# liyheng/MAGPO

Measured on AMD Instinct MI355X. Metric: env-steps/sec (all agents stepping jointly), CoordSum-4ag, full MAGPO update loop, higher is better.
Workload: dtype f32 (fp32 MFMA; as bf16 x3 operand splits = 24 mantissa bits, six products, fp32 accumulate: the GRU forward scan's recurrent GEMM)

## Files before the change

magpo_amd/csrc/seg_fused.hip:

```cpp
#include "fm_rows.hpp"

namespace magpo {

struct SegArgs {
  int tail;
  long R; int K;
  const float* r; const float* gp; long ldg; const float* gamma; const float* beta;
  const float* wo_t; const float* res; const float* s1; const float* s2;
  const float* pe; const int* pos; int npos;
  float* u; float* y; float* o; float* ope;
  const float* w0_t; const float* b0; float* out0; long ld0;
  const float* hs; const float* hw; const float* hb1; float* value;
  const float* q2_t[4]; float* q2[4]; int nq2;
  float* hn; const float* w1_t; const float* b1; float* logits;
  const int* rows;
};

__device__ __forceinline__ Row row_rms_reg(const Row& x, const Row& s) {
  Row q;
#pragma unroll
  for (int j = 0; j < 16; ++j) q.v[j] = x.v[j] * x.v[j];
  const float rstd = rsqrtf(row_sum(q) * (1.0f / 64.0f) + EPSN);
  Row r;
#pragma unroll
  for (int j = 0; j < 16; ++j) r.v[j] = x.v[j] * rstd * s.v[j];
  return r;
}

__device__ __forceinline__ Row dense64_reg(const Row& x, const float4 (&w)[4][4], const float* __restrict__ bias, int kq) {
  Row y;
#pragma unroll
  for (int g = 0; g < 4; ++g) {
    f32x4 acc = {0.f, 0.f, 0.f, 0.f};
#pragma unroll
    for (int gk = 0; gk < 4; ++gk) {
      acc = __builtin_amdgcn_mfma_f32_16x16x4f32(w[g][gk].x, x.v[4 * gk], acc, 0, 0, 0);
      acc = __builtin_amdgcn_mfma_f32_16x16x4f32(w[g][gk].y, x.v[4 * gk + 1], acc, 0, 0, 0);
      acc = __builtin_amdgcn_mfma_f32_16x16x4f32(w[g][gk].z, x.v[4 * gk + 2], acc, 0, 0, 0);
      acc = __builtin_amdgcn_mfma_f32_16x16x4f32(w[g][gk].w, x.v[4 * gk + 3], acc, 0, 0, 0);
    }
    float4 b = make_float4(0.f, 0.f, 0.f, 0.f);
    if (bias) b = ld4g(bias + 16 * g + 4 * kq);
    y.v[4 * g] = acc[0] + b.x; y.v[4 * g + 1] = acc[1] + b.y; y.v[4 * g + 2] = acc[2] + b.z; y.v[4 * g + 3] = acc[3] + b.w;
  }
  return y;
}
constexpr int WSP = 68;
__device__ __forceinline__ Row dense64_lds(const Row& x, const float* __restrict__ ws, int m, int kq) {
  Row y;
#pragma unroll
  for (int g = 0; g < 4; ++g) {
    f32x4 acc = {0.f, 0.f, 0.f, 0.f};
#pragma unroll
    for (int gk = 0; gk < 4; ++gk) {
      const float4 w = *reinterpret_cast<const float4*>(ws + (16 * g + m) * WSP + 16 * gk + 4 * kq);
      acc = __builtin_amdgcn_mfma_f32_16x16x4f32(w.x, x.v[4 * gk], acc, 0, 0, 0);
      acc = __builtin_amdgcn_mfma_f32_16x16x4f32(w.y, x.v[4 * gk + 1], acc, 0, 0, 0);
      acc = __builtin_amdgcn_mfma_f32_16x16x4f32(w.z, x.v[4 * gk + 2], acc, 0, 0, 0);
      acc = __builtin_amdgcn_mfma_f32_16x16x4f32(w.w, x.v[4 * gk + 3], acc, 0, 0, 0);
    }
    y.v[4 * g] = acc[0]; y.v[4 * g + 1] = acc[1]; y.v[4 * g + 2] = acc[2]; y.v[4 * g + 3] = acc[3];
  }
  return y;
}
__device__ __forceinline__ void load_w64(float4 (&w)[4][4], const float* __restrict__ Wt, int m, int kq) {
#pragma unroll
  for (int g = 0; g < 4; ++g)
#pragma unroll
    for (int gk = 0; gk < 4; ++gk) w[g][gk] = ld4g(Wt + (long)(16 * g + m) * AE + 16 * gk + 4 * kq);
}

template <int TAIL>
__global__ __launch_bounds__(64, 1) void k_seg_post(SegArgs a) {
  const int lane = threadIdx.x, m = lane & 15, kq = lane >> 4;
  const long ntiles = (a.R + 15) >> 4;
  float4 wo[4][4], w0[4][4], w0b[TAIL != 0 ? 4 : 1][4], w0c[TAIL == 2 ? 4 : 1][4];
  load_w64(wo, a.wo_t, m, kq);
  if (TAIL == 1 || TAIL == 3) load_w64(w0, a.w0_t, m, kq);
  if constexpr (TAIL == 1) { if (a.nq2 > 0) load_w64(w0b, a.q2_t[0], m, kq); }
  Row b1r;
  if constexpr (TAIL == 3) {
    load_w64(w0b, a.w1_t, m, kq);
#pragma unroll
    for (int j = 0; j < 16; ++j) { const int n = 16 * (j >> 2) + 4 * kq + (j & 3); b1r.v[j] = n < a.K ? a.b1[n] : 0.f; }
  }
  if (TAIL == 2) {
    load_w64(w0, a.w0_t, m, kq);
#pragma unroll
    for (int g = 0; g < 4; ++g)
#pragma unroll
      for (int gk = 0; gk < 4; ++gk) {
        w0b[g][gk] = ld4g(a.w0_t + (long)(64 + 16 * g + m) * AE + 16 * gk + 4 * kq);
        w0c[g][gk] = ld4g(a.w0_t + (long)(128 + 16 * g + m) * AE + 16 * gk + 4 * kq);
      }
  }
  const Row gam = row_load(a.gamma, kq), bet = row_load(a.beta, kq);
// ... 5 lines not shown
  const float hb1 = TAIL == 1 ? a.hb1[0] : 0.f;
  auto rowc = [&](long tile) { return min(tile * 16 + m, a.R - 1); };
  long tile = blockIdx.x;
  Row nr, ng, nres, npe;
  const bool want_pe = a.ope || TAIL == 1 || TAIL == 2;
  auto pe_row = [&](long row) {
    int p = a.pos[row];
    p = p < 0 ? 0 : (p >= a.npos ? a.npos - 1 : p);
    return row_load(a.pe + (long)p * AE, kq);
  };
  auto src_row = [&](long row) { return a.rows ? (long)a.rows[row] : row; };
  {
    const long row = rowc(tile), src = src_row(row);
    nr = row_load(a.r + row * AE, kq); ng = row_load(a.gp + src * a.ldg, kq); nres = row_load(a.res + src * AE, kq);
    if (want_pe) npe = pe_row(row);
  }
  for (; tile < ntiles; tile += gridDim.x) {
    const long row = tile * 16 + m;
    const long rw = min(row, a.R - 1);
    const Row r = nr, g = ng, res = nres, per = npe;
    {
      const long nrow = rowc(min(tile + (long)gridDim.x, ntiles - 1)), nsrc = src_row(nrow);
      nr = row_load(a.r + nrow * AE, kq); ng = row_load(a.gp + nsrc * a.ldg, kq); nres = row_load(a.res + nsrc * AE, kq);
      if (want_pe) npe = pe_row(nrow);
    }
    Row sq;
#pragma unroll
    for (int j = 0; j < 16; ++j) sq.v[j] = r.v[j] * r.v[j];
    const float mu = row_sum(r) * (1.0f / 64.0f), m2 = row_sum(sq) * (1.0f / 64.0f);
    const float rstd = rsqrtf(fmaxf(m2 - mu * mu, 0.f) + EPSN);
    Row u;
#pragma unroll
    for (int j = 0; j < 16; ++j) u.v[j] = fswish(g.v[j]) * ((r.v[j] - mu) * rstd * gam.v[j] + bet.v[j]);
    row_store(a.u + rw * AE, kq, u);
    const Row y = dense64_reg(u, wo, nullptr, kq);
    if (a.y) row_store(a.y + rw * AE, kq, y);
    Row o = row_add(res, y);
    {
      Row q;
#pragma unroll
      for (int j = 0; j < 16; ++j) q.v[j] = o.v[j] * o.v[j];
      const float rs = rsqrtf(row_sum(q) * (1.0f / 64.0f) + EPSN);
#pragma unroll
      for (int j = 0; j < 16; ++j) o.v[j] = o.v[j] * rs * s1.v[j];
    }
    if (a.s2) o = row_rms_reg(o, s2r);
    if (a.o) row_store(a.o + rw * AE, kq, o);
    Row ope = o;
    if (want_pe) {
      ope = row_add(o, per);
      if (a.ope) row_store(a.ope + rw * AE, kq, ope);
    }
    if (TAIL == 1) {
      const Row hv = row_add(dense64_reg(o, w0, nullptr, kq), b0r);
      row_store(a.out0 + rw * a.ld0, kq, hv);
      const Row hn = row_rms_reg(row_gelu(hv), hsr);
      Row hw;
#pragma unroll
      for (int j = 0; j < 16; ++j) hw.v[j] = hn.v[j] * hwr.v[j];
      const float val = row_sum(hw) + hb1;
      a.value[rw] = val;
      if constexpr (TAIL == 1) {
        if (a.nq2 > 0) row_store(a.q2[0] + rw * AE, kq, dense64_reg(ope, w0b, nullptr, kq));
      }
      for (int k = 1; k < a.nq2; ++k) {
        const Row q2 = dense64(ope, a.q2_t[k], nullptr, m, kq);
        row_store(a.q2[k] + rw * AE, kq, q2);
// ... 1 lines not shown
    } else if (TAIL == 2) {
      float* orow = a.out0 + rw * a.ld0;
      if constexpr (TAIL == 2) {
        row_store(orow, kq, dense64_reg(ope, w0, nullptr, kq));
        row_store(orow + 64, kq, dense64_reg(ope, w0b, nullptr, kq));
        row_store(orow + 128, kq, dense64_reg(ope, w0c, nullptr, kq));
      }
    } else if (TAIL == 3) {
      const Row hp = row_add(dense64_reg(o, w0, nullptr, kq), b0r);
      row_store(a.out0 + rw * a.ld0, kq, hp);
      const Row hn = row_rms_reg(row_gelu(hp), hsr);
      row_store(a.hn + rw * AE, kq, hn);
      if constexpr (TAIL == 3) {
        Row lg = row_add(dense64_reg(hn, w0b, nullptr, kq), b1r);
#pragma unroll
        for (int j = 0; j < 16; ++j) { const int n = 16 * (j >> 2) + 4 * kq + (j & 3); lg.v[j] = n < a.K ? lg.v[j] : 0.f; }
        row_store(a.logits + rw * AE, kq, lg);
      }
    }
  }
}


struct SegBwdArgs {
  long R;
  const float* a; const float* y; const float* s1; const float* s2;
  const float* d0; const float* d1; const float* d2;
  const float* wo_nat;
  const float* wo_t;
  const float* r; const float* gp; long ldg; const float* gamma; const float* beta;
  float* dsum; float* dr; float* dgp; long lddg;
  float* slab_s1; float* slab_s2; float* slab_ga; float* slab_be;
  const int* rows;
};

template <bool RECOMP>
__global__ __launch_bounds__(64, 1) void k_seg_bwd(SegBwdArgs a) {
  const int lane = threadIdx.x, m = lane & 15, kq = lane >> 4;
  const long ntiles = (a.R + 15) >> 4;
  float4 wo[4][4];
  __shared__ __align__(16) float wot[RECOMP ? 64 * WSP : 4];
  load_w64(wo, a.wo_nat, m, kq);
  constexpr bool recompute = RECOMP;
  if (recompute) {
    for (int i = lane; i < 64 * 16; i += 64) *reinterpret_cast<float4*>(&wot[(i >> 4) * WSP + 4 * (i & 15)]) = ld4g(a.wo_t + (i >> 4) * AE + 4 * (i & 15));
    __syncthreads();
  }
  __shared__ __align__(16) float prm[RECOMP ? 4 * 64 : 4];
  Row s1_, s2_, gam_, bet_;
  if (!RECOMP) {
    s1_ = row_load(a.s1, kq); gam_ = row_load(a.gamma, kq); bet_ = row_load(a.beta, kq);
    if (a.s2) s2_ = row_load(a.s2, kq);
  } else {
    prm[lane] = a.s1[lane]; prm[64 + lane] = a.s2 ? a.s2[lane] : 0.f; prm[128 + lane] = a.gamma[lane]; prm[192 + lane] = a.beta[lane];
    __syncthreads();
  }
  auto prow = [&](int which, const Row& reg) -> Row {
    if (!RECOMP) return reg;
    int off = which * 64 + 4 * kq;
    asm volatile("" : "+v"(off));
    Row r;
#pragma unroll
    for (int g = 0; g < 4; ++g) {
      const float4 t4 = *reinterpret_cast<const float4*>(&prm[off + 16 * g]);
      r.v[4 * g] = t4.x; r.v[4 * g + 1] = t4.y; r.v[4 * g + 2] = t4.z; r.v[4 * g + 3] = t4.w;
    }
    return r;
  };
  Row ds1, ds2, dga, dbe;
#pragma unroll
  for (int j = 0; j < 16; ++j) { ds1.v[j] = 0.f; ds2.v[j] = 0.f; dga.v[j] = 0.f; dbe.v[j] = 0.f; }
  auto rowc = [&](long tile) { return min(tile * 16 + m, a.R - 1); };
  Row na, ny, nd, nd1, nd2, nr, ng;
  auto fetch = [&](long row) {
    const long src = a.rows ? (long)a.rows[row] : row;
    na = row_load(a.a + src * AE, kq);
    if (a.y && !recompute) ny = row_load(a.y + row * AE, kq);
    nd = row_load(a.d0 + row * AE, kq);
    if (a.d1) nd1 = row_load(a.d1 + row * AE, kq);
    if (a.d2) nd2 = row_load(a.d2 + row * AE, kq);
    nr = row_load(a.r + row * AE, kq);
    ng = row_load(a.gp + src * a.ldg, kq);
  };
  long tile = blockIdx.x;
  fetch(rowc(tile));
  for (; tile < ntiles; tile += gridDim.x) {
    const long row = tile * 16 + m;
    const long rw = min(row, a.R - 1);
    const float live = row < a.R ? 1.f : 0.f;
    Row x = (a.y && !recompute) ? row_add(na, ny) : na;
    Row d = nd;
    if (a.d1) d = row_add(d, nd1);
    if (a.d2) d = row_add(d, nd2);
    const Row r = nr, g = ng;
    fetch(rowc(min(tile + (long)gridDim.x, ntiles - 1)));
    Row t;
#pragma unroll
    for (int j = 0; j < 16; ++j) t.v[j] = r.v[j] * r.v[j];
    const float mu = row_sum(r) * (1.0f / 64.0f), m2 = row_sum(t) * (1.0f / 64.0f);
    const float rstd = rsqrtf(fmaxf(m2 - mu * mu, 0.f) + EPSN);
    if (recompute) {
      const Row gam = prow(2, gam_), bet = prow(3, bet_);
      Row u;
#pragma unroll
      for (int j = 0; j < 16; ++j) u.v[j] = fswish(g.v[j]) * ((r.v[j] - mu) * rstd * gam.v[j] + bet.v[j]);
      x = row_add(x, dense64_lds(u, wot, m, kq));
    }
#pragma unroll
    for (int j = 0; j < 16; ++j) t.v[j] = x.v[j] * x.v[j];
    const float rstd1 = rsqrtf(row_sum(t) * (1.0f / 64.0f) + EPSN);
    Row xh1;
#pragma unroll
    for (int j = 0; j < 16; ++j) xh1.v[j] = x.v[j] * rstd1;
    const Row s1 = prow(0, s1_);
    if (a.s2) {
      const Row s2 = prow(1, s2_);
      Row y1;
#pragma unroll
      for (int j = 0; j < 16; ++j) { y1.v[j] = xh1.v[j] * s1.v[j]; t.v[j] = y1.v[j] * y1.v[j]; }
      const float rstd2 = rsqrtf(row_sum(t) * (1.0f / 64.0f) + EPSN);
#pragma unroll
      for (int j = 0; j < 16; ++j) {
        const float xh2 = y1.v[j] * rstd2;
        ds2.v[j] += live * d.v[j] * xh2;
        y1.v[j] = xh2;
        d.v[j] = d.v[j] * s2.v[j];
        t.v[j] = d.v[j] * xh2;
      }
      const float dot2 = row_sum(t) * (1.0f / 64.0f);
#pragma unroll
      for (int j = 0; j < 16; ++j) d.v[j] = (d.v[j] - y1.v[j] * dot2) * rstd2;
    }
#pragma unroll
    for (int j = 0; j < 16; ++j) {
      ds1.v[j] += live * d.v[j] * xh1.v[j];
      d.v[j] = d.v[j] * s1.v[j];
      t.v[j] = d.v[j] * xh1.v[j];
    }
    const float dot1 = row_sum(t) * (1.0f / 64.0f);
    Row dsum;
#pragma unroll
    for (int j = 0; j < 16; ++j) dsum.v[j] = (d.v[j] - xh1.v[j] * dot1) * rstd1;
    row_store(a.dsum + rw * AE, kq, dsum);
    const Row du = dense64_reg(dsum, wo, nullptr, kq);
    const Row gam = prow(2, gam_), bet = prow(3, bet_);
    Row xh, gg, dg;
#pragma unroll
    for (int j = 0; j < 16; ++j) {
      xh.v[j] = (r.v[j] - mu) * rstd;
      const float rn = xh.v[j] * gam.v[j] + bet.v[j];
      const float sg = fast_sigmoid(g.v[j]);
      const float sw = g.v[j] * sg;
      const float swg = sg * (1.0f + g.v[j] * (1.0f - sg));
      const float drn = du.v[j] * sw;
      dg.v[j] = du.v[j] * rn * swg;
      dga.v[j] += live * drn * xh.v[j];
      dbe.v[j] += live * drn;
      gg.v[j] = drn * gam.v[j];
      t.v[j] = gg.v[j] * xh.v[j];
    }
    const float mg = row_sum(gg) * (1.0f / 64.0f), mgx = row_sum(t) * (1.0f / 64.0f);
    Row dx;
#pragma unroll
    for (int j = 0; j < 16; ++j) dx.v[j] = (gg.v[j] - mg - xh.v[j] * mgx) * rstd;
    row_store(a.dr + rw * AE, kq, dx);
    row_store(a.dgp + rw * a.lddg, kq, dg);
  }
#pragma unroll
  for (int j = 0; j < 16; ++j) { ds1.v[j] = gsum(ds1.v[j], 16); ds2.v[j] = gsum(ds2.v[j], 16); dga.v[j] = gsum(dga.v[j], 16); dbe.v[j] = gsum(dbe.v[j], 16); }
  if (m == 0) {
    row_store(a.slab_s1 + (long)blockIdx.x * AE, kq, ds1);
    if (a.s2) row_store(a.slab_s2 + (long)blockIdx.x * AE, kq, ds2);
    row_store(a.slab_ga + (long)blockIdx.x * AE, kq, dga);
    row_store(a.slab_be + (long)blockIdx.x * AE, kq, dbe);
  }
}

}

using namespace magpo;

extern "C" int magpo_seg_post(const int* dims_host, long R, const void* const* p, int nptrs, hipStream_t st) {
  if (R <= 0) return MAGPO_OK;
  if (nptrs != 34) { set_error("magpo_seg_post: pointer table size mismatch"); return MAGPO_EINVAL; }
  SegArgs a;
  a.tail = dims_host[0]; a.K = dims_host[1]; a.npos = dims_host[2]; a.ldg = dims_host[3]; a.ld0 = dims_host[4]; a.nq2 = dims_host[5];
  a.R = R;
  if (a.tail < 0 || a.tail > 3 || a.nq2 < 0 || a.nq2 > 4 || a.K < 1 || a.K > 64) { set_error("magpo_seg_post: bad arguments"); return MAGPO_EINVAL; }
  int i = 0;
  a.r = (const float*)p[i++]; a.gp = (const float*)p[i++]; a.gamma = (const float*)p[i++]; a.beta = (const float*)p[i++];
  a.wo_t = (const float*)p[i++]; a.res = (const float*)p[i++]; a.s1 = (const float*)p[i++]; a.s2 = (const float*)p[i++];
  a.pe = (const float*)p[i++]; a.pos = (const int*)p[i++];
  a.u = (float*)p[i++]; a.y = (float*)p[i++]; a.o = (float*)p[i++]; a.ope = (float*)p[i++];
  a.w0_t = (const float*)p[i++]; a.b0 = (const float*)p[i++]; a.out0 = (float*)p[i++];
  a.hs = (const float*)p[i++]; a.hw = (const float*)p[i++]; a.hb1 = (const float*)p[i++]; a.value = (float*)p[i++];
  for (int k = 0; k < 4; ++k) a.q2_t[k] = (const float*)p[i++];
  for (int k = 0; k < 4; ++k) a.q2[k] = (float*)p[i++];
  a.hn = (float*)p[i++]; a.w1_t = (const float*)p[i++]; a.b1 = (const float*)p[i++]; a.logits = (float*)p[i++];
  a.rows = (const int*)p[i++];
  const long ntiles = (R + 15) / 16;
  long grid = 256 * 4;
  if (grid > ntiles) grid = ntiles;
  switch (a.tail) {
    case 0: hipLaunchKernelGGL(k_seg_post<0>, dim3((unsigned)grid), dim3(64), 0, st, a); break;
    case 1: hipLaunchKernelGGL(k_seg_post<1>, dim3((unsigned)grid), dim3(64), 0, st, a); break;
    case 2: hipLaunchKernelGGL(k_seg_post<2>, dim3((unsigned)grid), dim3(64), 0, st, a); break;
    default: hipLaunchKernelGGL(k_seg_post<3>, dim3((unsigned)grid), dim3(64), 0, st, a); break;
  }
  return check_launch("magpo_seg_post");
}

extern "C" int magpo_seg_bwd_grid(long R) { const long nt = (R + 15) / 16; return (int)(nt < 1024 ? (nt < 1 ? 1 : nt) : 1024); }

extern "C" int magpo_seg_bwd(long R, long ldg, long lddg, const void* const* p, int nptrs, hipStream_t st) {
  if (R <= 0) return MAGPO_OK;
  if (nptrs != 21) { set_error("magpo_seg_bwd: pointer table size mismatch"); return MAGPO_EINVAL; }
  SegBwdArgs a;
  a.R = R; a.ldg = ldg; a.lddg = lddg;
  int i = 0;
  a.a = (const float*)p[i++]; a.y = (const float*)p[i++]; a.s1 = (const float*)p[i++]; a.s2 = (const float*)p[i++];
  a.d0 = (const float*)p[i++]; a.d1 = (const float*)p[i++]; a.d2 = (const float*)p[i++]; a.wo_nat = (const float*)p[i++];
  a.r = (const float*)p[i++]; a.gp = (const float*)p[i++]; a.gamma = (const float*)p[i++]; a.beta = (const float*)p[i++];
  a.dsum = (float*)p[i++]; a.dr = (float*)p[i++]; a.dgp = (float*)p[i++];
  a.slab_s1 = (float*)p[i++]; a.slab_s2 = (float*)p[i++]; a.slab_ga = (float*)p[i++]; a.slab_be = (float*)p[i++];
  a.rows = (const int*)p[i++];
  a.wo_t = (const float*)p[i++];
  if (a.wo_t) hipLaunchKernelGGL(k_seg_bwd<true>, dim3((unsigned)magpo_seg_bwd_grid(R)), dim3(64), 0, st, a);
  else hipLaunchKernelGGL(k_seg_bwd<false>, dim3((unsigned)magpo_seg_bwd_grid(R)), dim3(64), 0, st, a);
  return check_launch("magpo_seg_bwd");
}
```

magpo_amd/sable.py:

```python
from __future__ import annotations

import math
from typing import Dict, Optional, Tuple

import numpy as np
import torch

from ._lib import lib
from .params import FlatParams, WidthEmbedding, guider_layout, guider_named_views, init_guider
from .tuning import Tuning

E = 64
TILE = 64
LW = 64


def decay_kappas(n_head: int, scaling: float):
    k = 1.0 - np.exp(np.linspace(np.log(np.float32(1 / 32)), np.log(np.float32(1 / 512)), n_head, dtype=np.float32))
    return [float(x) for x in (k.astype(np.float32) * np.float32(scaling)).astype(np.float32)]


class _Bufs:
    def __init__(self, device):
        self.device = device
# ... 415 lines not shown
                        v[d + "retn2.gn.scale"], v[d + "retn2.gn.bias"],
                        g(f"qkvg1_{k}", 4 * E), g(f"q2_{k}"), g(f"kvg2_{k}", 4 * E)]
            tabs = (np.array([N, A, K, F, nb, nh, self.hs, self.gs, self.npos, 1 if value_only else 0, self.Fld, self.tuning.act_envs_per_wave,
                              1 if pending else 0, 1 if flush else 0, 1 if precand else 0, 1 if defer else 0], dtype=np.int32),
                    np.array((self.kappas + [0.0] * 4)[:4], dtype=np.float32),
                    np.array([ptr(t) for t in glob], dtype=np.uint64), np.array([ptr(t) for t in blk], dtype=np.uint64))
            if len(self._act_tabs) > 4096:
                self._act_tabs.clear()
            self._act_tabs[cache_key] = tabs
        dims, kap, gp, bp = tabs
        keys = None
        if kdev is None and not value_only:
            keys = np.ascontiguousarray(np.asarray(sample_keys, dtype=np.uint32).reshape(A, 2))
        self.L.call("magpo_sable_act", dims.ctypes.data, kap.ctypes.data, None if keys is None else keys.ctypes.data,
                    gp.ctypes.data, int(gp.size), bp.ctypes.data, int(bp.size), self._st())

    get_actions = act_fused

    def _seg_post(self, tail, r, gp, ldg, gamma, beta, wo_t, res, s1, s2, pos, u, y, o, ope, R, w0_t=None, b0=None, out0=None, ld0=0,
                  hs=None, hw=None, hb1=None, value=None, q2_t=(), q2=(), hn=None, w1_t=None, b1=None, logits=None, rows=None):
        ptr = lambda t: 0 if t is None else t.data_ptr()
        q2_t, q2 = list(q2_t) + [None] * (4 - len(q2_t)), list(q2) + [None] * (4 - len(q2))
        tab = [r, gp, gamma, beta, wo_t, res, s1, s2, self.pe, pos, u, y, o, ope, w0_t, b0, out0, hs, hw, hb1, value, *q2_t, *q2, hn, w1_t, b1, logits, rows]
        key = (tail, R, tuple(ptr(t) for t in tab))
        ent = self._seg_tabs.get(key)
        if ent is None:
            nq2 = sum(1 for t in q2 if t is not None)
            ent = (np.array([tail, self.K, self.npos, ldg, ld0, nq2], dtype=np.int32), np.array([ptr(t) for t in tab], dtype=np.uint64))
            if len(self._seg_tabs) > 256:
                self._seg_tabs.clear()
            self._seg_tabs[key] = ent
        self.L.call("magpo_seg_post", ent[0].ctypes.data, R, ent[1].ctypes.data, int(ent[1].size), self._st())

    def _seg_bwd(self, a, y, s1, s2, d0, d1, d2, wo_nat, r, gp, ldg, pfx, dsum, dr, dgp, lddg, R, g_s1, g_s2, acc_s1=False, rows=None, wo_t=None):
        v, gv, b = self.v, self.gv, self.b
        ptr = lambda t: 0 if t is None else t.data_ptr()
        G = self.L.call("magpo_seg_bwd_grid", R)
        sl = [b.get(f"sb_{i}", (G, E)) for i in range(4)]
        tab = [a, y, s1, s2, d0, d1, d2, wo_nat, r, gp, v[pfx + "gn.scale"], v[pfx + "gn.bias"], dsum, dr, dgp, sl[0], sl[1] if s2 is not None else None, sl[2], sl[3], rows, wo_t]
        key = ("bwd", R, ldg, lddg, tuple(ptr(t) for t in tab))
        ent = self._seg_tabs.get(key)
        if ent is None:
            ent = np.array([ptr(t) for t in tab], dtype=np.uint64)
            self._seg_tabs[key] = ent
        self.L.call("magpo_seg_bwd", R, ldg, lddg, ent.ctypes.data, int(ent.size), self._st())
        self.reduce(sl[0], g_s1, accumulate=acc_s1)
        if s2 is not None:
            self.reduce(sl[1], g_s2)
        self.reduce(sl[2], gv[pfx + "gn.scale"]); self.reduce(sl[3], gv[pfx + "gn.bias"])

    def train_fwd(self, obs, prev_idx, pos, dones, s0, seq_env, nseq: int, T: int, classes=None):
        L, st, A, K, F, v, b, nb, E = self.L, self._st(), self.A, self.K, self.F, self.v, self.b, self.nb, self.E
        R = nseq * T * A
        g = lambda n, w=E: b.get("t_" + n, (R, w))
        direct = classes is not None and self.fused_segments
        self._saved = dict(obs=obs, prev_idx=prev_idx, pos=pos, dones=dones, nseq=nseq, T=T, R=R, classes=classes, direct=direct)
        rep, reppe, hv, value = g("rep"), g("reppe"), g("hv"), b.get("t_value", (R,))
        logits = b.get("t_logits", (R, LW), zero=True)
        if classes is not None:
            obs_c, pos_c = classes["rows"][0], classes["rows"][1]
            Ce = obs_c.shape[0]
            xn_c, kin_c, qkvg_c = b.get("c_xn0", (Ce, E)), b.get("c_kin0", (Ce, E)), b.get("c_qkvg0", (Ce, 4 * E))
            L.call("magpo_embed_fwd", 0, obs_c, F, F, v["enc.obs.norm.scale"], v["enc.obs.dense.kernel"], None, 0, v["enc.ln.scale"],
                   self.pe, pos_c, 1, self.npos, None, 0, xn_c, E, kin_c, E, Ce, E, st)
            self.lin(kin_c, E, self.wt["qkvg0"], None, qkvg_c, 4 * E, Ce, E, 4 * E)
            if not direct:
                L.call("magpo_gather_rows", xn_c, E, classes["enc"][0], g("xn0"), E, R, E, st)
                L.call("magpo_gather_rows", qkvg_c, 4 * E, classes["enc"][0], g("qkvg0", 4 * E), 4 * E, R, 4 * E, st)
        elif self.wide:
            on, z0 = b.get("t_on", (R, 128)), g("z0")
            L.call("magpo_obsnorm_fwd", obs, self.Fld, F, v["enc.obs.norm.scale"], on, R, st)
            self.lin(on, 128, self.wt["wobs"], None, z0, E, R, 128, E)
            L.call("magpo_headmid_fwd", z0, E, v["enc.ln.scale"], g("xn0"), E, None, None, None, 0, R, E, st)
            L.call("magpo_add_pe", g("xn0"), E, self.pe, pos, 1, self.npos, g("kin0"), E, R, E, st)
        else:
            L.call("magpo_embed_fwd", 0, obs, self.Fld, F, v["enc.obs.norm.scale"], v["enc.obs.dense.kernel"], None, 0, v["enc.ln.scale"],
                   self.pe, pos, 1, self.npos, None, 0, g("xn0"), E, g("kin0"), E, R, E, st)
        for k in range(nb):
            e = f"enc.block{k}."
            rows = classes["enc"][0] if direct and k == 0 else None
            if rows is not None:
                xn, qkvg = xn_c, qkvg_c
            else:
                xn, qkvg = g(f"xn{k}"), g(f"qkvg{k}", 4 * E)
            r, u = g(f"r{k}"), g(f"u{k}")
            y = None if self.fused_segments else g(f"y{k}")
            if k > 0 or classes is None:
                self.lin(g(f"kin{k}"), E, self.wt[f"qkvg{k}"], None, qkvg, 4 * E, R, E, 4 * E)
            self._ret_fwd(qkvg, 4 * E, qkvg[:, E:], 4 * E, qkvg[:, 2 * E:], 4 * E, r, s0[0][k], seq_env, dones, f"st_e{k}", nseq, T, 0, rows=rows)
            if self.fused_segments and k == nb - 1:
                self._seg_post(1, r, qkvg[:, 3 * E:], 4 * E, v[e + "retn.gn.scale"], v[e + "retn.gn.bias"], self.wt[f"wo{k}"], xn,
                               v[e + "ln1.scale"], v[e + "ln2.scale"], pos, u, y, rep, reppe, R, w0_t=self.wt["vh0"], b0=v["enc.head.dense0.bias"],
                               out0=hv, ld0=E, hs=v["enc.head.norm.scale"], hw=v["enc.head.dense1.kernel"], hb1=v["enc.head.dense1.bias"],
                               value=value, q2_t=[self.wt[f"q2{j}"] for j in range(nb)], q2=[g(f"q2{j}") for j in range(nb)], rows=rows)
                continue
            if self.fused_segments:
                repb = g(f"repb{k}")
                self._seg_post(0, r, qkvg[:, 3 * E:], 4 * E, v[e + "retn.gn.scale"], v[e + "retn.gn.bias"], self.wt[f"wo{k}"], xn,
                               v[e + "ln1.scale"], v[e + "ln2.scale"], pos, u, y, repb, None, R, rows=rows)
                L.call("magpo_resnorm_fwd", repb, E, None, 0, v["enc.ln.scale"], None, self.pe, pos, 1, self.npos,
                       g(f"xn{k + 1}"), E, g(f"kin{k + 1}"), E, R, E, st)
                continue
            self._retpost_fwd(r, qkvg[:, 3 * E:], 4 * E, v[e + "retn.gn.scale"], v[e + "retn.gn.bias"], u, R)
            self.lin(u, E, self.wt[f"wo{k}"], None, y, E, R, E, E)
            if k == nb - 1:
                L.call("magpo_resnorm_fwd", xn, E, y, E, v[e + "ln1.scale"], v[e + "ln2.scale"], self.pe, pos, 1, self.npos,
                       rep, E, reppe, E, R, E, st)
            else:
                repb = g(f"repb{k}")
                L.call("magpo_resnorm_fwd", xn, E, y, E, v[e + "ln1.scale"], v[e + "ln2.scale"], None, None, 0, 0, repb, E, None, 0, R, E, st)
                L.call("magpo_resnorm_fwd", repb, E, None, 0, v["enc.ln.scale"], None, self.pe, pos, 1, self.npos,
                       g(f"xn{k + 1}"), E, g(f"kin{k + 1}"), E, R, E, st)
        if not self.fused_segments:
            self.lin(rep, E, self.wt["vh0"], v["enc.head.dense0.bias"], hv, E, R, E, E)
            L.call("magpo_headmid_fwd", hv, E, v["enc.head.norm.scale"], None, 0, v["enc.head.dense1.kernel"], v["enc.head.dense1.bias"],
                   value, 1, R, E, st)
        if classes is not None:
            prev_c, posd_c = classes["rows"][2], classes["rows"][3]
            Cd = prev_c.shape[0]
            x_c, xpe_c, qkvg1_c = b.get("c_x0", (Cd, E)), b.get("c_xpe0", (Cd, E)), b.get("c_qkvg10", (Cd, 4 * E))
            L.call("magpo_embed_fwd", 1, None, 0, 0, None, v["dec.act.kernel"], prev_c, 1, v["dec.ln.scale"], self.pe, posd_c, 1, self.npos,
                   None, 0, x_c, E, xpe_c, E, Cd, E, st)
            self.lin(xpe_c, E, self.wt["qkvg10"], None, qkvg1_c, 4 * E, Cd, E, 4 * E)
            if not direct:
                L.call("magpo_gather_rows", x_c, E, classes["dec"][0], g("x0"), E, R, E, st)
                L.call("magpo_gather_rows", qkvg1_c, 4 * E, classes["dec"][0], g("qkvg10", 4 * E), 4 * E, R, 4 * E, st)
        else:
            L.call("magpo_embed_fwd", 1, None, 0, 0, None, v["dec.act.kernel"], prev_idx, 1, v["dec.ln.scale"], self.pe, pos, 1, self.npos,
                   None, 0, g("x0"), E, g("xpe0"), E, R, E, st)
        for k in range(nb):
            d = f"dec.block{k}."
            rows = classes["dec"][0] if direct and k == 0 else None
            if rows is not None:
                x, qkvg1 = x_c, qkvg1_c
            else:
                x, qkvg1 = g(f"x{k}"), g(f"qkvg1{k}", 4 * E)
            r1, u1 = g(f"r1{k}"), g(f"u1{k}")
            cpe, q2, kvg2, r2, u2 = g(f"cpe{k}"), g(f"q2{k}"), g(f"kvg2{k}", 3 * E), g(f"r2{k}"), g(f"u2{k}")
            y1, y2 = (None, None) if self.fused_segments else (g(f"y1{k}"), g(f"y2{k}"))
            if k > 0 or classes is None:
                self.lin(g(f"xpe{k}"), E, self.wt[f"qkvg1{k}"], None, qkvg1, 4 * E, R, E, 4 * E)
            self._ret_fwd(qkvg1, 4 * E, qkvg1[:, E:], 4 * E, qkvg1[:, 2 * E:], 4 * E, r1, s0[1][k], seq_env, dones, f"st_1{k}", nseq, T, 1, rows=rows)
            if self.fused_segments:
                self._seg_post(2, r1, qkvg1[:, 3 * E:], 4 * E, v[d + "retn1.gn.scale"], v[d + "retn1.gn.bias"], self.wt[f"wo1{k}"], x,
                               v[d + "ln1.scale"], None, pos, u1, y1, None, cpe, R, w0_t=self.wt[f"kvg2{k}"], out0=kvg2, ld0=3 * E, rows=rows)
                self._ret_fwd(q2, E, kvg2, 3 * E, kvg2[:, E:], 3 * E, r2, s0[2][k], seq_env, dones, f"st_2{k}", nseq, T, 1)
                if k == nb - 1:
                    self._seg_post(3, r2, kvg2[:, 2 * E:], 3 * E, v[d + "retn2.gn.scale"], v[d + "retn2.gn.bias"], self.wt[f"wo2{k}"], rep,
                                   v[d + "ln2.scale"], v[d + "ln3.scale"], pos, u2, y2, g(f"x{nb}"), None, R, w0_t=self.wt["h0"],
                                   b0=v["dec.head.dense0.bias"], out0=g("hp"), ld0=E, hs=v["dec.head.norm.scale"], hn=g("hn"),
                                   w1_t=self.wt["h1"], b1=v["dec.head.dense1.bias"], logits=logits)
                else:
                    self._seg_post(0, r2, kvg2[:, 2 * E:], 3 * E, v[d + "retn2.gn.scale"], v[d + "retn2.gn.bias"], self.wt[f"wo2{k}"], rep,
                                   v[d + "ln2.scale"], v[d + "ln3.scale"], pos, u2, y2, g(f"x{k + 1}"), g(f"xpe{k + 1}"), R)
                continue
            self._retpost_fwd(r1, qkvg1[:, 3 * E:], 4 * E, v[d + "retn1.gn.scale"], v[d + "retn1.gn.bias"], u1, R)
            self.lin(u1, E, self.wt[f"wo1{k}"], None, y1, E, R, E, E)
            L.call("magpo_resnorm_fwd", x, E, y1, E, v[d + "ln1.scale"], None, self.pe, pos, 1, self.npos, None, 0, cpe, E, R, E, st)
            self.lin(reppe, E, self.wt[f"q2{k}"], None, q2, E, R, E, E)
            self.lin(cpe, E, self.wt[f"kvg2{k}"], None, kvg2, 3 * E, R, E, 3 * E)
            self._ret_fwd(q2, E, kvg2, 3 * E, kvg2[:, E:], 3 * E, r2, s0[2][k], seq_env, dones, f"st_2{k}", nseq, T, 1)
            self._retpost_fwd(r2, kvg2[:, 2 * E:], 3 * E, v[d + "retn2.gn.scale"], v[d + "retn2.gn.bias"], u2, R)
            self.lin(u2, E, self.wt[f"wo2{k}"], None, y2, E, R, E, E)
            if k == nb - 1:
                L.call("magpo_resnorm_fwd", rep, E, y2, E, v[d + "ln2.scale"], v[d + "ln3.scale"], None, None, 0, 0, g(f"x{nb}"), E,
                       None, 0, R, E, st)
            else:
                L.call("magpo_resnorm_fwd", rep, E, y2, E, v[d + "ln2.scale"], v[d + "ln3.scale"], self.pe, pos, 1, self.npos,
                       g(f"x{k + 1}"), E, g(f"xpe{k + 1}"), E, R, E, st)
        if not self.fused_segments:
            hp, hn = g("hp"), g("hn")
            self.lin(g(f"x{nb}"), E, self.wt["h0"], v["dec.head.dense0.bias"], hp, E, R, E, E)
            L.call("magpo_headmid_fwd", hp, E, v["dec.head.norm.scale"], hn, E, None, None, None, 0, R, E, st)
            self.lin(hn, E, self.wt["h1"], v["dec.head.dense1.bias"], logits, LW, R, E, K)
        return logits, value

    def train_bwd(self, dlogits, dvalue):
        L, st, A, K, F, v, gv, b, nb, E = self.L, self._st(), self.A, self.K, self.F, self.v, self.gv, self.b, self.nb, self.E
        sv = self._saved
        R, nseq, T = sv["R"], sv["nseq"], sv["T"]
        obs, prev_idx, pos, dones = sv["obs"], sv["prev_idx"], sv["pos"], sv["dones"]
        cl, Rd = sv["classes"], R
        t = lambda n: b.t["t_" + n]
        g = lambda n, w=E: b.get("g_" + n, (R, w))
        grid = L.call("magpo_row_grid", R)
        slab = lambda n, w=E: b.get("s_" + n, (grid, w))
        self.wgrad(t("hn"), E, dlogits, LW, R, E, K, gv["dec.head.dense1.kernel"], gv["dec.head.dense1.bias"])
        dhn = g("dhn")
        self.lin(dlogits, LW, self.wt["h1_nat_pad"], None, dhn, E, R, LW, E)
        dhp = g("dhp_l")
        L.call("magpo_headmid_bwd", t("hp"), E, v["dec.head.norm.scale"], dhn, E, None, None, 0, dhp, E, slab("a"), None, None, R, E, st)
        self.reduce(slab("a"), gv["dec.head.norm.scale"])
        self.wgrad(t(f"x{nb}"), E, dhp, E, R, E, E, gv["dec.head.dense0.kernel"], gv["dec.head.dense0.bias"])
        dout = g("dout")
        self.lin(dhp, E, v["dec.head.dense0.kernel"], None, dout, E, R, E, E)
        din0, din1 = dout, None
        drep_q, drep_r = None, None
        for k in reversed(range(nb)):
            d = f"dec.block{k}."
            dsum2 = g(f"dsum2_{k}")
            dr2 = g("dr"); dq2 = g(f"dq2_{k}"); dkvg2 = g(f"dkvg2_{k}", 3 * E)
            kvg2 = t(f"kvg2{k}")
            if self.fused_segments:
                self._seg_bwd(t("rep"), None, v[d + "ln2.scale"], v[d + "ln3.scale"], din0, din1, None, v[d + "retn2.w_o"], t(f"r2{k}"),
                              kvg2[:, 2 * E:], 3 * E, d + "retn2.", dsum2, dr2, dkvg2[:, 2 * E:], 3 * E, R, gv[d + "ln2.scale"], gv[d + "ln3.scale"],
                              wo_t=self.wt[f"wo2{k}"])
                self.wgrad(t(f"u2{k}"), E, dsum2, E, R, E, E, gv[d + "retn2.w_o"])
            else:
                L.call("magpo_resnorm_bwd", t("rep"), E, t(f"y2{k}"), E, v[d + "ln2.scale"], v[d + "ln3.scale"], din0, E, din1, E if din1 is not None else 0,
                       None, 0, dsum2, E, slab("a"), slab("b"), R, E, st)
                self.reduce(slab("a"), gv[d + "ln2.scale"]); self.reduce(slab("b"), gv[d + "ln3.scale"])
                self.wgrad(t(f"u2{k}"), E, dsum2, E, R, E, E, gv[d + "retn2.w_o"])
                du2 = g("du")
                self.lin(dsum2, E, v[d + "retn2.w_o"], None, du2, E, R, E, E)
                self._retpost_bwd(t(f"r2{k}"), kvg2[:, 2 * E:], 3 * E, d + "retn2.", du2, dr2, dkvg2[:, 2 * E:], 3 * E, R, slab("a"), slab("b"))
            self._ret_bwd(t(f"q2{k}"), E, kvg2, 3 * E, kvg2[:, E:], 3 * E, dr2, dq2, E, dkvg2, 3 * E, dkvg2[:, E:], 3 * E, dones,
                          f"st_2{k}", nseq, T, 1)
            self.wgrad(t("reppe"), E, dq2, E, R, E, E, gv[d + "retn2.w_q"])
            self.wgrad(t(f"cpe{k}"), E, dkvg2, 3 * E, R, E, 3 * E, gv[d + "retn2.w_kvg"])
            dreppe = g(f"dreppe_{k}"); dcpe = g("dcpe")
            self.lin(dq2, E, v[d + "retn2.w_q"], None, dreppe, E, R, E, E)
            self.lin(dkvg2, 3 * E, v[d + "retn2.w_kvg"], None, dcpe, E, R, 3 * E, E)
            if drep_q is None:
                drep_q, drep_r = dreppe, dsum2
            else:
                self.add_(drep_q, dreppe); self.add_(drep_r, dsum2)
            dsum1 = g(f"dsum1_{k}")
            dr1 = g("dr"); dqkvg1 = g(f"dqkvg1_{k}", 4 * E)
            rows = cl["dec"][0] if sv["direct"] and k == 0 else None
            qkvg1, xk = (b.t["c_qkvg10"], b.t["c_x0"]) if rows is not None else (t(f"qkvg1{k}"), t(f"x{k}"))
            if self.fused_segments:
                self._seg_bwd(xk, None, v[d + "ln1.scale"], None, dcpe, None, None, v[d + "retn1.w_o"], t(f"r1{k}"),
                              qkvg1[:, 3 * E:], 4 * E, d + "retn1.", dsum1, dr1, dqkvg1[:, 3 * E:], 4 * E, R, gv[d + "ln1.scale"], None, rows=rows,
                              wo_t=self.wt[f"wo1{k}"])
                self.wgrad(t(f"u1{k}"), E, dsum1, E, R, E, E, gv[d + "retn1.w_o"])
            else:
                L.call("magpo_resnorm_bwd", t(f"x{k}"), E, t(f"y1{k}"), E, v[d + "ln1.scale"], None, dcpe, E, None, 0, None, 0, dsum1, E,
                       slab("a"), None, R, E, st)
                self.reduce(slab("a"), gv[d + "ln1.scale"])
                self.wgrad(t(f"u1{k}"), E, dsum1, E, R, E, E, gv[d + "retn1.w_o"])
                du1 = g("du")
                self.lin(dsum1, E, v[d + "retn1.w_o"], None, du1, E, R, E, E)
                self._retpost_bwd(t(f"r1{k}"), qkvg1[:, 3 * E:], 4 * E, d + "retn1.", du1, dr1, dqkvg1[:, 3 * E:], 4 * E, R, slab("a"), slab("b"))
            self._ret_bwd(qkvg1, 4 * E, qkvg1[:, E:], 4 * E, qkvg1[:, 2 * E:], 4 * E, dr1, dqkvg1, 4 * E, dqkvg1[:, E:], 4 * E,
                          dqkvg1[:, 2 * E:], 4 * E, dones, f"st_1{k}", nseq, T, 1, rows=rows)
            if k == 0 and cl is not None:
                _, order, offsets = cl["dec"]
                Cd = cl["rows"][2].shape[0]
                dq_c, ds_c = b.get("gc_dqkvg1", (Cd, 4 * E)), b.get("gc_dsum1", (Cd, E))
                part = b.get("gc_part_d", (L.call("magpo_class_sum_slots", Cd), Cd, 4 * E))
                L.call("magpo_class_sum", dqkvg1, 4 * E, order, offsets, Cd, 4 * E, part, dq_c, st)
                L.call("magpo_class_sum", dsum1, E, order, offsets, Cd, E, part, ds_c, st)
                self.wgrad(b.t["c_xpe0"], E, dq_c, 4 * E, Cd, E, 4 * E, gv[d + "retn1.w_qkvg"])
                dkin1 = b.get("gc_dkin1", (Cd, E))
                self.lin_dx_qkvg(dq_c, d + "retn1.w_qkvg", dkin1, Cd)
                din0, din1, prev_idx, Rd = ds_c, dkin1, cl["rows"][2], Cd
                break
            self.wgrad(t(f"xpe{k}"), E, dqkvg1, 4 * E, R, E, 4 * E, gv[d + "retn1.w_qkvg"])
            dkin1 = g(f"dkin1_{k}")
            self.lin_dx_qkvg(dqkvg1, d + "retn1.w_qkvg", dkin1, R)
            din0, din1 = dsum1, dkin1
        gridd = L.call("magpo_row_grid", Rd)
        sa_d, sw_d = b.get("s_a_d", (gridd, E)), b.get("s_w_d", (gridd, 32 * E))
        L.call("magpo_embed_bwd", 1, None, 0, din0, E, din1, E, None, 0, v["dec.ln.scale"], None, 0, sa_d, sw_d,
               K + 1, None, 0, 0, None, v["dec.act.kernel"], None, prev_idx, 1, Rd, E, st)
        self.reduce(sa_d, gv["dec.ln.scale"])
        self.reduce(sw_d, gv["dec.act.kernel"], P=(K + 1) * E, stride=32 * E)
        dhv = g("dhv")
        L.call("magpo_headmid_bwd", t("hv"), E, v["enc.head.norm.scale"], None, 0, v["enc.head.dense1.kernel"], dvalue, 1, dhv, E,
               slab("a"), slab("b"), slab("c", 1), R, E, st)
        self.reduce(slab("a"), gv["enc.head.norm.scale"]); self.reduce(slab("b"), gv["enc.head.dense1.kernel"])
        self.reduce(slab("c", 1), gv["enc.head.dense1.bias"], P=1, stride=1)
        self.wgrad(t("rep"), E, dhv, E, R, E, E, gv["enc.head.dense0.kernel"], gv["enc.head.dense0.bias"])
        drep_v = g("dout")
        self.lin(dhv, E, v["enc.head.dense0.kernel"], None, drep_v, E, R, E, E)
        e0, e1, e2 = drep_v, drep_q, drep_r
        first_ln = True
        for k in reversed(range(nb)):
            e = f"enc.block{k}."
            dsum0 = g(f"dsum0_{k}")
            dr = g("dr"); dqkvg = g(f"dqkvg_{k}", 4 * E)
            rows = cl["enc"][0] if sv["direct"] and k == 0 else None
            qkvg, xnk = (b.t["c_qkvg0"], b.t["c_xn0"]) if rows is not None else (t(f"qkvg{k}"), t(f"xn{k}"))
            if self.fused_segments:
                self._seg_bwd(xnk, None, v[e + "ln1.scale"], v[e + "ln2.scale"], e0, e1, e2, v[e + "retn.w_o"], t(f"r{k}"),
                              qkvg[:, 3 * E:], 4 * E, e + "retn.", dsum0, dr, dqkvg[:, 3 * E:], 4 * E, R, gv[e + "ln1.scale"], gv[e + "ln2.scale"], rows=rows,
                              wo_t=self.wt[f"wo{k}"])
                self.wgrad(t(f"u{k}"), E, dsum0, E, R, E, E, gv[e + "retn.w_o"])
            else:
                L.call("magpo_resnorm_bwd", t(f"xn{k}"), E, t(f"y{k}"), E, v[e + "ln1.scale"], v[e + "ln2.scale"], e0, E, e1, E if e1 is not None else 0,
                       e2, E if e2 is not None else 0, dsum0, E, slab("a"), slab("b"), R, E, st)
                self.reduce(slab("a"), gv[e + "ln1.scale"]); self.reduce(slab("b"), gv[e + "ln2.scale"])
                self.wgrad(t(f"u{k}"), E, dsum0, E, R, E, E, gv[e + "retn.w_o"])
                du = g("du")
                self.lin(dsum0, E, v[e + "retn.w_o"], None, du, E, R, E, E)
                self._retpost_bwd(t(f"r{k}"), qkvg[:, 3 * E:], 4 * E, e + "retn.", du, dr, dqkvg[:, 3 * E:], 4 * E, R, slab("a"), slab("b"))
            self._ret_bwd(qkvg, 4 * E, qkvg[:, E:], 4 * E, qkvg[:, 2 * E:], 4 * E, dr, dqkvg, 4 * E, dqkvg[:, E:], 4 * E, dqkvg[:, 2 * E:], 4 * E,
                          dones, f"st_e{k}", nseq, T, 0, rows=rows)
            if k == 0 and cl is not None:
                _, order, offsets = cl["enc"]
                obs_c = cl["rows"][0]
                Ce = obs_c.shape[0]
                dq_c, ds_c = b.get("gc_dqkvg0", (Ce, 4 * E)), b.get("gc_dsum0", (Ce, E))
                part = b.get("gc_part_e", (L.call("magpo_class_sum_slots", Ce), Ce, 4 * E))
                L.call("magpo_class_sum", dqkvg, 4 * E, order, offsets, Ce, 4 * E, part, dq_c, st)
                L.call("magpo_class_sum", dsum0, E, order, offsets, Ce, E, part, ds_c, st)
                self.wgrad(b.t["c_kin0"], E, dq_c, 4 * E, Ce, E, 4 * E, gv[e + "retn.w_qkvg"])
                dkin = b.get("gc_dkin0", (Ce, E))
                self.lin_dx_qkvg(dq_c, e + "retn.w_qkvg", dkin, Ce)
                gride = L.call("magpo_row_grid", Ce)
                sa, sw, sd = b.get("s_a_e", (gride, E)), b.get("s_w_e", (gride, 32 * E)), b.get("s_d_e", (gride, 32))
                L.call("magpo_embed_bwd", 0, None, 0, ds_c, E, dkin, E, None, 0, v["enc.ln.scale"], None, 0, sa, sw, F,
                       obs_c, F, F, v["enc.obs.norm.scale"], v["enc.obs.dense.kernel"], sd, None, 0, Ce, E, st)
                self.reduce(sa, gv["enc.ln.scale"], accumulate=not first_ln)
                self.reduce(sd, gv["enc.obs.norm.scale"], P=F, stride=32)
                self.reduce(sw, gv["enc.obs.dense.kernel"], P=F * E, stride=32 * E)
                break
            self.wgrad(t(f"kin{k}"), E, dqkvg, 4 * E, R, E, 4 * E, gv[e + "retn.w_qkvg"])
            dkin = g(f"dkin_{k}")
            self.lin_dx_qkvg(dqkvg, e + "retn.w_qkvg", dkin, R)
            if k > 0:
# ... 31 lines not shown
```

Before: 4.067 million.

## Fuse retention output-projection weight gradient into segment backward kernel

The segment backward kernel now accumulates dW_o per block with MFMA from the recomputed gated activation u and dsum, staged through LDS, and writes per-block slabs that are then reduced. This removes the separate wgrad GEMM and the forward-pass stores and reloads of u, which the forward kernel now skips when fused segments are on. Both W_o orientations move into a fragment-ordered LDS layout so register pressure stays low. The cost is extra LDS syncs per tile, 16 accumulator fragments held in registers, and a slab reduction of G×64×64.

```diff
diff --git a/magpo_amd/csrc/seg_fused.hip b/magpo_amd/csrc/seg_fused.hip
--- a/magpo_amd/csrc/seg_fused.hip
+++ b/magpo_amd/csrc/seg_fused.hip
@@ -45,15 +45,14 @@
   }
   return y;
 }
-constexpr int WSP = 68;
-__device__ __forceinline__ Row dense64_lds(const Row& x, const float* __restrict__ ws, int m, int kq) {
+__device__ __forceinline__ Row dense64_flds(const Row& x, const float* __restrict__ wf, int off) {
   Row y;
 #pragma unroll
   for (int g = 0; g < 4; ++g) {
     f32x4 acc = {0.f, 0.f, 0.f, 0.f};
 #pragma unroll
     for (int gk = 0; gk < 4; ++gk) {
-      const float4 w = *reinterpret_cast<const float4*>(ws + (16 * g + m) * WSP + 16 * gk + 4 * kq);
+      const float4 w = *reinterpret_cast<const float4*>(wf + (4 * g + gk) * 256 + off);
       acc = __builtin_amdgcn_mfma_f32_16x16x4f32(w.x, x.v[4 * gk], acc, 0, 0, 0);
       acc = __builtin_amdgcn_mfma_f32_16x16x4f32(w.y, x.v[4 * gk + 1], acc, 0, 0, 0);
       acc = __builtin_amdgcn_mfma_f32_16x16x4f32(w.z, x.v[4 * gk + 2], acc, 0, 0, 0);
@@ -62,6 +61,12 @@
     y.v[4 * g] = acc[0]; y.v[4 * g + 1] = acc[1]; y.v[4 * g + 2] = acc[2]; y.v[4 * g + 3] = acc[3];
   }
   return y;
+}
+__device__ __forceinline__ void fill_flds(float* __restrict__ wf, const float* __restrict__ Wt, int lane) {
+  const int m = lane & 15, kq = lane >> 4;
+#pragma unroll
+  for (int f = 0; f < 16; ++f)
+    *reinterpret_cast<float4*>(wf + f * 256 + 4 * lane) = ld4g(Wt + (long)(16 * (f >> 2) + m) * AE + 16 * (f & 3) + 4 * kq);
 }
 __device__ __forceinline__ void load_w64(float4 (&w)[4][4], const float* __restrict__ Wt, int m, int kq) {
 #pragma unroll
@@ -133,7 +138,7 @@
     Row u;
 #pragma unroll
     for (int j = 0; j < 16; ++j) u.v[j] = fswish(g.v[j]) * ((r.v[j] - mu) * rstd * gam.v[j] + bet.v[j]);
-    row_store(a.u + rw * AE, kq, u);
+    if (a.u) row_store(a.u + rw * AE, kq, u);
     const Row y = dense64_reg(u, wo, nullptr, kq);
     if (a.y) row_store(a.y + rw * AE, kq, y);
     Row o = row_add(res, y);
@@ -201,19 +206,44 @@
   float* dsum; float* dr; float* dgp; long lddg;
   float* slab_s1; float* slab_s2; float* slab_ga; float* slab_be;
   const int* rows;
+  float* slab_wo;
 };
 
-template <bool RECOMP>
+constexpr int TSP = 68;
+__device__ __forceinline__ void tile_stage(float* __restrict__ stg, const Row& x, float scale, int m, int kq) {
+  lsync();
+#pragma unroll
+  for (int g = 0; g < 4; ++g)
+    *reinterpret_cast<float4*>(stg + m * TSP + 16 * g + 4 * kq) =
+        make_float4(x.v[4 * g] * scale, x.v[4 * g + 1] * scale, x.v[4 * g + 2] * scale, x.v[4 * g + 3] * scale);
+  lsync();
+}
+__device__ __forceinline__ void tile_kstep(const float* __restrict__ stg, int s, int m, int kq, float (&t)[4]) {
+#pragma unroll
+  for (int b = 0; b < 4; ++b) t[b] = stg[(4 * kq + s) * TSP + 16 * b + m];
+}
+
+template <bool RECOMP, bool WGRAD = false>
 __global__ __launch_bounds__(64, 1) void k_seg_bwd(SegBwdArgs a) {
+  static_assert(RECOMP || !WGRAD, "dW_o needs the recomputed u");
   const int lane = threadIdx.x, m = lane & 15, kq = lane >> 4;
   const long ntiles = (a.R + 15) >> 4;
-  float4 wo[4][4];
-  __shared__ __align__(16) float wot[RECOMP ? 64 * WSP : 4];
-  load_w64(wo, a.wo_nat, m, kq);
+  float4 wo[RECOMP ? 1 : 4][4];
+  __shared__ __align__(16) float wot[RECOMP ? 64 * 64 : 4];
+  __shared__ __align__(16) float won[RECOMP ? 64 * 64 : 4];
+  __shared__ __align__(16) float stg[WGRAD ? 16 * TSP : 4];
+  if constexpr (!RECOMP) load_w64(wo, a.wo_nat, m, kq);
   constexpr bool recompute = RECOMP;
   if (recompute) {
-    for (int i = lane; i < 64 * 16; i += 64) *reinterpret_cast<float4*>(&wot[(i >> 4) * WSP + 4 * (i & 15)]) = ld4g(a.wo_t + (i >> 4) * AE + 4 * (i & 15));
+    fill_flds(wot, a.wo_t, lane); fill_flds(won, a.wo_nat, lane);
     __syncthreads();
+  }
+  f32x4 dwo[WGRAD ? 4 : 1][WGRAD ? 4 : 1];
+  if constexpr (WGRAD) {
+#pragma unroll
+    for (int bi = 0; bi < 4; ++bi)
+#pragma unroll
+      for (int bo = 0; bo < 4; ++bo) dwo[bi][bo] = f32x4{0.f, 0.f, 0.f, 0.f};
   }
   __shared__ __align__(16) float prm[RECOMP ? 4 * 64 : 4];
   Row s1_, s2_, gam_, bet_;
@@ -268,12 +298,20 @@
     for (int j = 0; j < 16; ++j) t.v[j] = r.v[j] * r.v[j];
     const float mu = row_sum(r) * (1.0f / 64.0f), m2 = row_sum(t) * (1.0f / 64.0f);
     const float rstd = rsqrtf(fmaxf(m2 - mu * mu, 0.f) + EPSN);
+    float ut[4][4];
     if (recompute) {
       const Row gam = prow(2, gam_), bet = prow(3, bet_);
       Row u;
 #pragma unroll
       for (int j = 0; j < 16; ++j) u.v[j] = fswish(g.v[j]) * ((r.v[j] - mu) * rstd * gam.v[j] + bet.v[j]);
-      x = row_add(x, dense64_lds(u, wot, m, kq));
+      int woff = 4 * lane;
+      asm volatile("" : "+v"(woff));
+      x = row_add(x, dense64_flds(u, wot, woff));
+      if constexpr (WGRAD) {
+        tile_stage(stg, u, 1.0f, m, kq);
+#pragma unroll
+        for (int s = 0; s < 4; ++s) tile_kstep(stg, s, m, kq, ut[s]);
+      }
     }
 #pragma unroll
     for (int j = 0; j < 16; ++j) t.v[j] = x.v[j] * x.v[j];
@@ -311,7 +349,27 @@
 #pragma unroll
     for (int j = 0; j < 16; ++j) dsum.v[j] = (d.v[j] - xh1.v[j] * dot1) * rstd1;
     row_store(a.dsum + rw * AE, kq, dsum);
-    const Row du = dense64_reg(dsum, wo, nullptr, kq);
+    if constexpr (WGRAD) {
+      tile_stage(stg, dsum, live, m, kq);
+      float dt[4][4];
+#pragma unroll
+      for (int s = 0; s < 4; ++s) tile_kstep(stg, s, m, kq, dt[s]);
+#pragma unroll
+      for (int s = 0; s < 4; ++s)
+#pragma unroll
+        for (int bi = 0; bi < 4; ++bi)
+#pragma unroll
+          for (int bo = 0; bo < 4; ++bo)
+            dwo[bi][bo] = __builtin_amdgcn_mfma_f32_16x16x4f32(dt[s][bo], ut[s][bi], dwo[bi][bo], 0, 0, 0);
+    }
+    Row du;
+    if constexpr (RECOMP) {
+      int woff = 4 * lane;
+      asm volatile("" : "+v"(woff));
+      du = dense64_flds(dsum, won, woff);
+    } else {
+      du = dense64_reg(dsum, wo, nullptr, kq);
+    }
     const Row gam = prow(2, gam_), bet = prow(3, bet_);
     Row xh, gg, dg;
 #pragma unroll
@@ -342,6 +400,14 @@
     if (a.s2) row_store(a.slab_s2 + (long)blockIdx.x * AE, kq, ds2);
     row_store(a.slab_ga + (long)blockIdx.x * AE, kq, dga);
     row_store(a.slab_be + (long)blockIdx.x * AE, kq, dbe);
+  }
+  if constexpr (WGRAD) {
+    float* sw = a.slab_wo + (long)blockIdx.x * (AE * AE);
+#pragma unroll
+    for (int bi = 0; bi < 4; ++bi)
+#pragma unroll
+      for (int bo = 0; bo < 4; ++bo)
+        st4g(sw + (16 * bi + m) * AE + 16 * bo + 4 * kq, make_float4(dwo[bi][bo][0], dwo[bi][bo][1], dwo[bi][bo][2], dwo[bi][bo][3]));
   }
 }
 
@@ -383,7 +449,8 @@
 
 extern "C" int magpo_seg_bwd(long R, long ldg, long lddg, const void* const* p, int nptrs, hipStream_t st) {
   if (R <= 0) return MAGPO_OK;
-  if (nptrs != 21) { set_error("magpo_seg_bwd: pointer table size mismatch"); return MAGPO_EINVAL; }
+  if (nptrs != 21 && nptrs != 22) { set_error("magpo_seg_bwd: pointer table size mismatch"); return MAGPO_EINVAL; }
+  if (nptrs == 22 && p[21] && !p[20]) { set_error("magpo_seg_bwd: the dW_o slab needs wo_t (u is only formed when y is recomputed)"); return MAGPO_EINVAL; }
   SegBwdArgs a;
   a.R = R; a.ldg = ldg; a.lddg = lddg;
   int i = 0;
@@ -394,7 +461,9 @@
   a.slab_s1 = (float*)p[i++]; a.slab_s2 = (float*)p[i++]; a.slab_ga = (float*)p[i++]; a.slab_be = (float*)p[i++];
   a.rows = (const int*)p[i++];
   a.wo_t = (const float*)p[i++];
-  if (a.wo_t) hipLaunchKernelGGL(k_seg_bwd<true>, dim3((unsigned)magpo_seg_bwd_grid(R)), dim3(64), 0, st, a);
+  a.slab_wo = nptrs == 22 ? (float*)p[i++] : nullptr;
+  if (a.slab_wo) hipLaunchKernelGGL((k_seg_bwd<true, true>), dim3((unsigned)magpo_seg_bwd_grid(R)), dim3(64), 0, st, a);
+  else if (a.wo_t) hipLaunchKernelGGL(k_seg_bwd<true>, dim3((unsigned)magpo_seg_bwd_grid(R)), dim3(64), 0, st, a);
   else hipLaunchKernelGGL(k_seg_bwd<false>, dim3((unsigned)magpo_seg_bwd_grid(R)), dim3(64), 0, st, a);
   return check_launch("magpo_seg_bwd");
 }
diff --git a/magpo_amd/sable.py b/magpo_amd/sable.py
--- a/magpo_amd/sable.py
+++ b/magpo_amd/sable.py
@@ -471,12 +471,16 @@
             self._seg_tabs[key] = ent
         self.L.call("magpo_seg_post", ent[0].ctypes.data, R, ent[1].ctypes.data, int(ent[1].size), self._st())
 
-    def _seg_bwd(self, a, y, s1, s2, d0, d1, d2, wo_nat, r, gp, ldg, pfx, dsum, dr, dgp, lddg, R, g_s1, g_s2, acc_s1=False, rows=None, wo_t=None):
+    def _seg_bwd(self, a, y, s1, s2, d0, d1, d2, wo_nat, r, gp, ldg, pfx, dsum, dr, dgp, lddg, R, g_s1, g_s2, acc_s1=False, rows=None, wo_t=None,
+                 g_wo=None):
         v, gv, b = self.v, self.gv, self.b
         ptr = lambda t: 0 if t is None else t.data_ptr()
         G = self.L.call("magpo_seg_bwd_grid", R)
         sl = [b.get(f"sb_{i}", (G, E)) for i in range(4)]
         tab = [a, y, s1, s2, d0, d1, d2, wo_nat, r, gp, v[pfx + "gn.scale"], v[pfx + "gn.bias"], dsum, dr, dgp, sl[0], sl[1] if s2 is not None else None, sl[2], sl[3], rows, wo_t]
+        if g_wo is not None:
+            sl_wo = b.get("sb_wo", (G, E * E))
+            tab.append(sl_wo)
         key = ("bwd", R, ldg, lddg, tuple(ptr(t) for t in tab))
         ent = self._seg_tabs.get(key)
         if ent is None:
@@ -487,6 +491,8 @@
         if s2 is not None:
             self.reduce(sl[1], g_s2)
         self.reduce(sl[2], gv[pfx + "gn.scale"]); self.reduce(sl[3], gv[pfx + "gn.bias"])
+        if g_wo is not None:
+            self.reduce(sl_wo, g_wo)
 
     def train_fwd(self, obs, prev_idx, pos, dones, s0, seq_env, nseq: int, T: int, classes=None):
         L, st, A, K, F, v, b, nb, E = self.L, self._st(), self.A, self.K, self.F, self.v, self.b, self.nb, self.E
@@ -522,7 +528,7 @@
                 xn, qkvg = xn_c, qkvg_c
             else:
                 xn, qkvg = g(f"xn{k}"), g(f"qkvg{k}", 4 * E)
-            r, u = g(f"r{k}"), g(f"u{k}")
+            r, u = g(f"r{k}"), None if self.fused_segments else g(f"u{k}")
             y = None if self.fused_segments else g(f"y{k}")
             if k > 0 or classes is None:
                 self.lin(g(f"kin{k}"), E, self.wt[f"qkvg{k}"], None, qkvg, 4 * E, R, E, 4 * E)
@@ -574,9 +580,8 @@
                 x, qkvg1 = x_c, qkvg1_c
             else:
                 x, qkvg1 = g(f"x{k}"), g(f"qkvg1{k}", 4 * E)
-            r1, u1 = g(f"r1{k}"), g(f"u1{k}")
-            cpe, q2, kvg2, r2, u2 = g(f"cpe{k}"), g(f"q2{k}"), g(f"kvg2{k}", 3 * E), g(f"r2{k}"), g(f"u2{k}")
-            y1, y2 = (None, None) if self.fused_segments else (g(f"y1{k}"), g(f"y2{k}"))
+            r1, cpe, q2, kvg2, r2 = g(f"r1{k}"), g(f"cpe{k}"), g(f"q2{k}"), g(f"kvg2{k}", 3 * E), g(f"r2{k}")
+            u1, u2, y1, y2 = (None,) * 4 if self.fused_segments else (g(f"u1{k}"), g(f"u2{k}"), g(f"y1{k}"), g(f"y2{k}"))
             if k > 0 or classes is None:
                 self.lin(g(f"xpe{k}"), E, self.wt[f"qkvg1{k}"], None, qkvg1, 4 * E, R, E, 4 * E)
             self._ret_fwd(qkvg1, 4 * E, qkvg1[:, E:], 4 * E, qkvg1[:, 2 * E:], 4 * E, r1, s0[1][k], seq_env, dones, f"st_1{k}", nseq, T, 1, rows=rows)
@@ -643,8 +648,7 @@
             if self.fused_segments:
                 self._seg_bwd(t("rep"), None, v[d + "ln2.scale"], v[d + "ln3.scale"], din0, din1, None, v[d + "retn2.w_o"], t(f"r2{k}"),
                               kvg2[:, 2 * E:], 3 * E, d + "retn2.", dsum2, dr2, dkvg2[:, 2 * E:], 3 * E, R, gv[d + "ln2.scale"], gv[d + "ln3.scale"],
-                              wo_t=self.wt[f"wo2{k}"])
-                self.wgrad(t(f"u2{k}"), E, dsum2, E, R, E, E, gv[d + "retn2.w_o"])
+                              wo_t=self.wt[f"wo2{k}"], g_wo=gv[d + "retn2.w_o"])
             else:
                 L.call("magpo_resnorm_bwd", t("rep"), E, t(f"y2{k}"), E, v[d + "ln2.scale"], v[d + "ln3.scale"], din0, E, din1, E if din1 is not None else 0,
                        None, 0, dsum2, E, slab("a"), slab("b"), R, E, st)
@@ -671,8 +675,7 @@
             if self.fused_segments:
                 self._seg_bwd(xk, None, v[d + "ln1.scale"], None, dcpe, None, None, v[d + "retn1.w_o"], t(f"r1{k}"),
                               qkvg1[:, 3 * E:], 4 * E, d + "retn1.", dsum1, dr1, dqkvg1[:, 3 * E:], 4 * E, R, gv[d + "ln1.scale"], None, rows=rows,
-                              wo_t=self.wt[f"wo1{k}"])
-                self.wgrad(t(f"u1{k}"), E, dsum1, E, R, E, E, gv[d + "retn1.w_o"])
+                              wo_t=self.wt[f"wo1{k}"], g_wo=gv[d + "retn1.w_o"])
             else:
                 L.call("magpo_resnorm_bwd", t(f"x{k}"), E, t(f"y1{k}"), E, v[d + "ln1.scale"], None, dcpe, E, None, 0, None, 0, dsum1, E,
                        slab("a"), None, R, E, st)
@@ -724,8 +727,7 @@
             if self.fused_segments:
                 self._seg_bwd(xnk, None, v[e + "ln1.scale"], v[e + "ln2.scale"], e0, e1, e2, v[e + "retn.w_o"], t(f"r{k}"),
                               qkvg[:, 3 * E:], 4 * E, e + "retn.", dsum0, dr, dqkvg[:, 3 * E:], 4 * E, R, gv[e + "ln1.scale"], gv[e + "ln2.scale"], rows=rows,
-                              wo_t=self.wt[f"wo{k}"])
-                self.wgrad(t(f"u{k}"), E, dsum0, E, R, E, E, gv[e + "retn.w_o"])
+                              wo_t=self.wt[f"wo{k}"], g_wo=gv[e + "retn.w_o"])
             else:
                 L.call("magpo_resnorm_bwd", t(f"xn{k}"), E, t(f"y{k}"), E, v[e + "ln1.scale"], v[e + "ln2.scale"], e0, E, e1, E if e1 is not None else 0,
                        e2, E if e2 is not None else 0, dsum0, E, slab("a"), slab("b"), R, E, st)
```

After: 4.122 million, median of 6. 1.01x the previous value.
